# sailor-z/3DAHV

Measured on AMD Instinct MI355X. Metric: rotation hypotheses scored/sec (B=1), higher is better.
Workload: dtype f32; 1 GPU; CO3D pair (BASELINE.json configs[1]): B=1, ONE set of N_hyp=50000 Haar rotations split over the GPUs (contiguous shards, n_offset), source volume 16x8x8x8 (P=512 voxel sites x 16 ch), head 384->32->32, 64 positions; n_hyp_per_gpu=50000, n_hyp_total=50000, parallelism=hypothesis axis sharded x1, 8-byte key all-reduce(max), backend=single process, lanes=1

## Files before the change

### 3dahv_amd/_lib.py

```python
from __future__ import annotations

import ctypes
import os
import subprocess

_HERE = os.path.dirname(os.path.abspath(__file__))
CSRC = os.path.join(_HERE, "csrc")
LIB_PATH = os.path.join(CSRC, "libahv_hip.so")

AHV_SCORE_RESET_BEST = 1
AHV_SCORE_SPLIT_F16 = 2
AHV_SCORE_NO_TEAMS = 4
AHV_SCORE_SPARE_CUS_SHIFT = 8
AHV_SELECT_RESET_KEY = 1
AHV_KEY_EMPTY = -(1 << 63)
AHV_TOPK_MAX_K = 64
AHV_TOPK_RESET_LIST = 1
AHV_SO3_MAX_LADDER = 8
AHV_POSTERIOR_MAX_MODES = 16
AHV_POSTERIOR_RESET_STATE = 1
AHV_VIEWS_MAX = 16
AHV_VIEWS_RESET_BEST = 1
AHV_VIEWS_NO_ANGLE_LIMIT = 2
AHV_VIEW_SLOT_EXCLUDED = -1
AHV_VIEW_SLOT_OVERFLOW = -2

_vp = ctypes.c_void_p
_i64 = ctypes.c_int64
# ... 73 lines not shown
SIGNATURES["ahv_fuse_view_scores_compact_f32"] = (_int, [_vp, _vp, _vp, _int, _int, _i64, _i64, _i64, _vp, _vp, _u32, _vp])
SIGNATURES["ahv_resample_workspace_bytes"] = (ctypes.c_size_t, [_int, _i64])
SIGNATURES["ahv_resample_f32"] = (_int, [_vp, _int, _i64, ctypes.c_float, _i64, _vp, _vp, _vp, ctypes.c_size_t, _u32, _vp])
SIGNATURES["ahv_compose_rotations_indexed_f32"] = (_int, [_vp, _vp, _i64, _i64, _vp, _i64, _int, _vp, _vp])
SIGNATURES["ahv_diffuse_rotations_f32"] = (_int, [_vp, _vp, _i64, _i64, _vp, _i64, _i64, _int, ctypes.c_uint64, _vp, ctypes.c_float,
                                                  ctypes.c_float, _vp, _vp, _vp])
SIGNATURES["ahv_predict_rotations_f32"] = (_int, [_vp, _vp, _i64, _vp, _i64, _i64, _vp, _i64, _i64, _int, ctypes.c_uint64, _vp]
                                           + [ctypes.c_float] * 5 + [_int, _vp, _vp, _vp, _vp])
SIGNATURES["ahv_track_advance"] = (_int, [ctypes.c_uint64, _vp, _int, _vp, _vp])
SIGNATURES["ahv_smooth_step_f32"] = (_int, [_vp, _vp, _vp, _vp, _i64, _int, _i64, _i64] + [ctypes.c_float] * 4 + [_vp] * 5)
SIGNATURES["ahv_smooth_backtrace_f32"] = (_int, [_vp, _vp, _vp, _vp, _i64, _int, _i64, _i64, _i64, _vp, _vp, _vp])

DIAG_SIGNATURES = {
    "ahv_score_hypotheses_clocked_f32": SIGNATURES.pop("ahv_score_hypotheses_clocked_f32"),
    "ahv_diag_score_plan": (_int, [_int, _i64, _u32, ctypes.POINTER(_int), ctypes.POINTER(_int), ctypes.POINTER(_i64)]),
}

_lib = None


class AhvError(RuntimeError):
    """A libahv_hip call returned a negative status."""


def build(force: bool = False) -> str:
    args = ["make", "-C", CSRC, "-j4"] + (["-B"] if force else [])
    proc = subprocess.run(args, stdout=subprocess.PIPE, stderr=subprocess.STDOUT, text=True)
    if proc.returncode != 0:
        raise RuntimeError("building libahv_hip.so failed:\n" + proc.stdout)
    return LIB_PATH
# ... 26 lines not shown
```

### 3dahv_amd/csrc/ahv_abi.hip

```cpp
#include <hip/hip_runtime.h>

#include <cstdarg>
#include <cstdio>
#include <cstring>

#include "../../include/ahv.h"
#include "../../include/ahv_diag.h"
#include "ahv_launch.h"

namespace ahv {
hipError_t launch_unpack_best(const int64_t*, int, float*, int64_t*, hipStream_t);
hipError_t launch_rotate_volume(const float*, int64_t, const float*, int64_t, int, int, int, int, float*, int,
                                hipStream_t);
hipError_t launch_rotate_volume_backward(const float*, int64_t, const float*, int64_t, int, int, int, int, float*, int,
                                         hipStream_t);
hipError_t launch_forward_3d2d(const float*, const float*, const float*, const float*, int64_t, float*, int,
                               hipStream_t);
hipError_t launch_score_features(const float*, const float*, int, int64_t, float*, int, hipStream_t);
hipError_t launch_argmax(const float*, int, int64_t, int64_t, int64_t*, int, hipStream_t);
hipError_t launch_fill_keys(int64_t*, int, hipStream_t);
int topk_parts(int64_t N);
hipError_t launch_topk(const float*, int, int64_t, int64_t, int, int64_t*, int64_t*, bool, hipStream_t);
hipError_t launch_topk_merge(const int64_t*, int, int, int, int64_t*, bool, hipStream_t);
hipError_t launch_select_topk(int64_t*, int, const float*, int64_t, int64_t, int64_t, int, float*, float*, int64_t*, bool,
// ... 96 lines not shown

int ahv_device_cu_count(void)
{
    const int cu = cu_count();
    if (cu < 0) return fail(AHV_EDEVICE, "no usable HIP device");
    return cu;
}

static hipError_t zero_span(void* p, size_t bytes, hipStream_t s)
{
    void* const ptrs[1] = {p};
    const size_t n[1] = {bytes};
    return ahv::launch_zero_fill(ptrs, n, 1, s);
}

static int score_common(const char* who, const float* vol_src, const float* tgt, bool tgt_is_volume, const float* R,
                        int64_t r_batch_stride, int64_t n_offset, const float* W1, const float* W2, const float* b2, int B,
                        int64_t N, float* scores, int64_t* best_key, float* feat_tgt_out, unsigned flags,
                        uint64_t* clock_stamps, void* stream)
{
    if (B < 0 || N < 0) return fail(AHV_EINVAL, "%s: negative size (B=%d, N=%lld)", who, B, (long long)N);
    if (B > 0 && N > 0 && (!vol_src || !tgt || !R || !W1 || !W2 || !b2))
        return fail(AHV_EINVAL, "%s: null input pointer", who);
    if (r_batch_stride != 0 && r_batch_stride < N * 9)
        return fail(AHV_EINVAL, "%s: r_batch_stride %lld must be 0 or >= N*9", who, (long long)r_batch_stride);
    if (n_offset < 0 || n_offset + N > 4294967296ll)
        return fail(AHV_EINVAL, "%s: n_offset + N must fit in 32 bits", who);
    if (flags & ~(AHV_SCORE_RESET_BEST | AHV_SCORE_SPLIT_F16 | AHV_SCORE_NO_TEAMS | AHV_SCORE_SPARE_CUS_MASK))
        return fail(AHV_EINVAL, "%s: unknown flags 0x%x", who, flags);
    const bool split = (flags & AHV_SCORE_SPLIT_F16) != 0;
    hipStream_t s = static_cast<hipStream_t>(stream);
    if (best_key && (flags & AHV_SCORE_RESET_BEST) && B > 0) {
        hipError_t e = ahv::launch_fill_keys(best_key, B, s);
        if (e != hipSuccess) return hip_fail("score: key reset", e);
    }
    const int cu = cu_count();
    if (cu < 0) return fail(AHV_EDEVICE, "no usable HIP device");
    if (tgt_is_volume && split) {
        if (B > 0 && !feat_tgt_out)
            return fail(AHV_EINVAL, "%s: AHV_SCORE_SPLIT_F16 needs feat_tgt_out (the target features go through it)", who);
        if (B > 0) {
            hipError_t e = ahv::launch_forward_3d2d(tgt, W1, W2, b2, B, feat_tgt_out, cu, s);
            if (e != hipSuccess) return hip_fail("verify_pair: forward_3d2d launch", e);
        }
        tgt = feat_tgt_out;
        tgt_is_volume = false;
        feat_tgt_out = nullptr;
    }
    if (B == 0) return AHV_OK;
    if (N == 0 && !(tgt_is_volume && feat_tgt_out)) return AHV_OK;
    ahv::ScoreLaunch a;
    a.vol_src = vol_src; a.tgt = tgt; a.tgt_is_volume = tgt_is_volume; a.R = R;
    a.r_batch_stride = r_batch_stride; a.n_offset = n_offset; a.W1 = W1; a.W2 = W2; a.b2 = b2; a.B = B; a.N = N;
    a.scores = scores; a.best_key = best_key; a.feat_tgt_out = feat_tgt_out; a.num_cu = cu;
    a.spare_cu = (int)((flags & AHV_SCORE_SPARE_CUS_MASK) >> AHV_SCORE_SPARE_CUS_SHIFT);
    a.split_f16 = split; a.no_teams = (flags & AHV_SCORE_NO_TEAMS) != 0; a.clock_stamps = clock_stamps;
    hipError_t e = ahv::launch_score_hypotheses(a, s);
    if (e != hipSuccess) return hip_fail("score: launch", e);
    return AHV_OK;
}

int ahv_score_hypotheses_f32(const float* vol_src, const float* feat_tgt, const float* R,
                             int64_t r_batch_stride, int64_t n_offset, const float* W1, const float* W2,
                             const float* b2, int B, int64_t N, float* scores, int64_t* best_key,
                             unsigned flags, void* stream)
{
    return score_common("score", vol_src, feat_tgt, false, R, r_batch_stride, n_offset, W1, W2, b2, B, N, scores, best_key,
                        nullptr, flags, nullptr, stream);
}

int ahv_score_hypotheses_clocked_f32(const float* vol_src, const float* feat_tgt, const float* R,
// ... 5 lines not shown
    return score_common("score_clocked", vol_src, feat_tgt, false, R, r_batch_stride, n_offset, W1, W2, b2, B, N, scores,
                        best_key, nullptr, flags, clock_stamps, stream);
}

int ahv_diag_score_plan(int B, int64_t N, unsigned flags, int* gx, int* gy, int64_t* n_main)
{
    if (B < 1 || N < 0) return fail(AHV_EINVAL, "score_plan: bad shape (B=%d, N=%lld)", B, (long long)N);
    const int cu = cu_count();
    if (cu < 0) return fail(AHV_EDEVICE, "no usable HIP device");
    const bool teams = !(flags & AHV_SCORE_SPLIT_F16) && !(flags & AHV_SCORE_NO_TEAMS);
    const ahv::ScorePlan p = ahv::plan_score_launch(B, N, cu, (int)((flags & AHV_SCORE_SPARE_CUS_MASK) >> AHV_SCORE_SPARE_CUS_SHIFT), teams);
    if (gx) *gx = p.gx;
    if (gy) *gy = p.gy;
    if (n_main) *n_main = p.n_main;
    return AHV_OK;
}

int ahv_verify_pair_f32(const float* vol_src, const float* vol_tgt, const float* R, int64_t r_batch_stride,
                        int64_t n_offset, const float* W1, const float* W2, const float* b2, int B, int64_t N,
                        float* scores, int64_t* best_key, float* feat_tgt_out, unsigned flags, uint64_t* clock_stamps,
                        void* stream)
{
    return score_common("verify_pair", vol_src, vol_tgt, true, R, r_batch_stride, n_offset, W1, W2, b2, B, N, scores,
                        best_key, feat_tgt_out, flags, clock_stamps, stream);
}

int ahv_unpack_best(const int64_t* best_key, int B, float* best_score, int64_t* best_idx, void* stream)
{
    if (!best_key) return fail(AHV_EINVAL, "unpack: null best_key");
    if (B < 0) return fail(AHV_EINVAL, "unpack: negative B");
// ... 102 lines not shown

int ahv_coarse_to_fine_f32(const float* vol_src, const float* vol_tgt, const float* R, int64_t r_batch_stride, int64_t N,
                           const float* D, int64_t N2, const float* W1, const float* W2, const float* b2, int B,
                           float* scores_coarse, float* scores_fine, int64_t* keys, uint32_t* sync, float* feat_tgt_out,
                           float* R_pred, float* fine_score, int64_t* fine_idx, float* coarse_score, int64_t* coarse_idx,
                           unsigned flags, void* stream)
{
    if (B < 0 || N < 0 || N2 < 0) return fail(AHV_EINVAL, "coarse_to_fine: negative size (B=%d, N=%lld, N2=%lld)", B, (long long)N, (long long)N2);
    if (B == 0) return AHV_OK;
    if (N == 0 || N2 == 0) return fail(AHV_EINVAL, "coarse_to_fine: empty hypothesis set (N=%lld, N2=%lld)", (long long)N, (long long)N2);
    if (!vol_src || !vol_tgt || !R || !D || !W1 || !W2 || !b2) return fail(AHV_EINVAL, "coarse_to_fine: null input pointer");
    if (!keys || !sync) return fail(AHV_EINVAL, "coarse_to_fine: keys and sync are required (2 B keys, 2 B + 1 counters)");
    if (r_batch_stride != 0 && r_batch_stride < N * 9)
        return fail(AHV_EINVAL, "coarse_to_fine: r_batch_stride %lld must be 0 or >= N*9", (long long)r_batch_stride);
    if (N > 4294967296ll || N2 > 4294967296ll) return fail(AHV_EINVAL, "coarse_to_fine: indices must fit in 32 bits");
    if (flags & ~(AHV_SCORE_NO_TEAMS | AHV_SCORE_SPARE_CUS_MASK)) return fail(AHV_EINVAL, "coarse_to_fine: unknown flags 0x%x", flags);
    const int cu = cu_count();
    if (cu < 0) return fail(AHV_EDEVICE, "no usable HIP device");
    ahv::CoarseToFineLaunch a;
    ahv::ScoreLaunch& c = a.coarse;
    c.vol_src = vol_src; c.tgt = vol_tgt; c.tgt_is_volume = true; c.R = R; c.r_batch_stride = r_batch_stride; c.n_offset = 0;
    c.W1 = W1; c.W2 = W2; c.b2 = b2; c.B = B; c.N = N; c.scores = scores_coarse; c.best_key = keys;
    c.feat_tgt_out = feat_tgt_out; c.num_cu = cu;
    c.spare_cu = (int)((flags & AHV_SCORE_SPARE_CUS_MASK) >> AHV_SCORE_SPARE_CUS_SHIFT);
    c.split_f16 = false; c.no_teams = (flags & AHV_SCORE_NO_TEAMS) != 0; c.clock_stamps = nullptr;
    a.D = D; a.N2 = N2; a.scores2 = scores_fine; a.best_key2 = keys + B; a.sync = sync; a.R_pred = R_pred;
    a.fine_score = fine_score; a.coarse_score = coarse_score; a.fine_idx = fine_idx; a.coarse_idx = coarse_idx;
    hipError_t e = ahv::launch_coarse_to_fine(a, static_cast<hipStream_t>(stream));
    if (e != hipSuccess) return hip_fail("coarse_to_fine: launch", e);
    return AHV_OK;
}

int ahv_reset_best(int64_t* best_key, int B, void* stream)
{
    if (B < 0) return fail(AHV_EINVAL, "reset_best: negative B");
    if (B == 0) return AHV_OK;
    if (!best_key) return fail(AHV_EINVAL, "reset_best: null best_key");
    hipError_t e = ahv::launch_fill_keys(best_key, B, static_cast<hipStream_t>(stream));
    if (e != hipSuccess) return hip_fail("reset_best: launch", e);
    return AHV_OK;
// ... 746 lines not shown
```

### 3dahv_amd/csrc/ahv_launch.h

```cpp
#pragma once
#include <hip/hip_runtime.h>
#include <stdint.h>

namespace ahv {

struct ScoreLaunch {
    const float* vol_src;
    const float* tgt;
    bool tgt_is_volume;
    const float* R;
    int64_t r_batch_stride, n_offset;
    const float *W1, *W2, *b2;
    int B;
    int64_t N;
    float* scores;
    int64_t* best_key;
    float* feat_tgt_out;
    int num_cu, spare_cu;
    bool split_f16;
    bool no_teams;
    uint64_t* clock_stamps;
};

struct ScorePlan {
    int gx, gy;
    int64_t n_main;
};

ScorePlan plan_score_launch(int B, int64_t N, int num_cu, int spare_cu, bool teams);
hipError_t launch_score_hypotheses(const ScoreLaunch& a, hipStream_t stream);
hipError_t launch_score_hypotheses_train(const ScoreLaunch& a, float* u_out, hipStream_t stream);

struct CoarseToFineLaunch {
    ScoreLaunch coarse;
    const float* D;
    int64_t N2;
    float* scores2;
    int64_t* best_key2;
    uint32_t* sync;
    float* R_pred;
    float *fine_score, *coarse_score;
// ... 6 lines not shown
```

### 3dahv_amd/csrc/ahv_score.hip

```cpp
#define AHV_FP32_LOW_HALF
#include "ahv_dual.h"
#include "ahv_split.h"
#include "ahv_team.h"
#include "ahv_exact.h"
#include "ahv_launch.h"

namespace ahv {

__device__ __forceinline__ int opaque(int x)
{
    asm volatile("" : "+v"(x));
    return x;
}

__device__ __forceinline__ float swap_add32(float a, float b)
{
    const auto r = __builtin_amdgcn_permlane32_swap(__float_as_uint(a), __float_as_uint(b), false, false);
    return __uint_as_float(r[0]) + __uint_as_float(r[1]);
}

__device__ __forceinline__ float swap_add16(float a, float b)
{
    const auto r = __builtin_amdgcn_permlane16_swap(__float_as_uint(a), __float_as_uint(b), false, false);
    return __uint_as_float(r[0]) + __uint_as_float(r[1]);
// ... 147 lines not shown
            for (int m2 = 0; m2 < 2; ++m2)
                tg[t][m2] = *reinterpret_cast<const f32x4*>(lds_src + ((2 * t + m2) * 64 + lane) * kSrcStride + 16);
        const float s = hyp_score_rs<SPLIT || kFp32LowHalf>(v, tg, lane);
        if (scores_b != nullptr && lane == 0) scores_b[he] = s;
        const key_t key = pack_key(s, (unsigned)(n_offset + he));
        best = key > best ? key : best;
    }
    return best;
}

template <bool SPLIT, bool TGT, bool C2F, bool SAVE_U = false>
__device__ __forceinline__ void score_hypotheses_body(
    const float* __restrict__ vol_src, const float* __restrict__ tgt, const float* __restrict__ R,
    long r_batch_stride, long n_offset, const float* __restrict__ W1, const float* __restrict__ W2,
    const float* __restrict__ b2, int B, long N, long n_main, float* __restrict__ scores,
    key_t* __restrict__ best_key, float* __restrict__ feat_tgt_out, unsigned long long* __restrict__ clk, const C2fArgs& cf)
{
    static_assert(!(SPLIT && TGT), "the split-f16 kernel takes ready-made target features");
    static_assert(!C2F || (TGT && !SPLIT), "the two-stage launch is the fp32 verify kernel");
    static_assert(!SAVE_U || (!SPLIT && !TGT && !C2F), "u is saved by the fp32 scorer with ready-made target features");
    if constexpr (!SPLIT) asm volatile("" ::: "v255");
    __shared__ __attribute__((aligned(1024))) float lds_src[kSrcFloats];
    __shared__ __attribute__((aligned(16))) float lds_w1[kW1TableFloats];
    __shared__ __attribute__((aligned(16))) float lds_q[8 * kQuarterFloats];
    __shared__ TeamSync lds_team;
    __shared__ NonFinite lds_nf;
    __shared__ unsigned long long lds_t_entry[2];
    if (clk != nullptr && threadIdx.x == 0) {
        lds_t_entry[0] = __builtin_amdgcn_s_memrealtime();
        lds_t_entry[1] = __builtin_amdgcn_s_memtime();
    }
    const int tid = threadIdx.x;
// ... 248 lines not shown
                best = score_share_exact<SPLIT>(lds_src, lds_w1, buf, W1, W2, b2, Rb, ec, N_s, h0, hstep, sc_b, n_offset_s, best, lane);
            } else {
                best = score_share_exact<SPLIT>(lds_src, lds_w1, buf, W1, W2, b2, Rb, NoCompose{}, N_s, h0, hstep, sc_b, n_offset_s, best, lane);
            }
            if constexpr (SPLIT) split_load_resident(w1res, reinterpret_cast<const f16x8*>(lds_w1), lane);
            if constexpr (SAVE_U) {
                const f32x4 qn = f32x4{__builtin_nanf(""), __builtin_nanf(""), __builtin_nanf(""), __builtin_nanf("")};
                for (long he = h0; he < N_s; he += hstep) {
                    float* uo = feat_tgt_out + ((long)b * N_s + he) * 2048 + lane * 4;
#pragma unroll
                    for (int i = 0; i < 8; ++i) *reinterpret_cast<f32x4*>(uo + i * 256) = qn;
                }
            }
        } else {
        if constexpr (!SPLIT && !SAVE_U) score_remainder_by_teams();
        long h = (long)wave * gridDim.x + residue;
        float Rn = h < n_main_s ? Rb[h * 9 + rl] : 0.0f;
#ifdef AHV_STAMPS
        unsigned long long tsum[11] = {0, 0, 0, 0, 0, 0, 0, 0, 0, 0, 0};
#endif
        for (; h < n_main_s; h += hstep) {
            float Rm[9];
#pragma unroll
            for (int i = 0; i < 9; ++i) Rm[i] = __builtin_bit_cast(float, __builtin_amdgcn_readlane(__builtin_bit_cast(int, Rn), i));
            hyp_rotation(Rm, st1);
            {
                const long hn = (h + hstep < n_main_s) ? h + hstep : h;
                Rn = Rb[hn * 9 + rl];
            }
            f32x4 acc[2][4];
#pragma unroll
            for (int m = 0; m < 2; ++m)
#pragma unroll
                for (int t = 0; t < 4; ++t) acc[m][t] = f32x4{0.f, 0.f, 0.f, 0.f};

#ifdef AHV_STAMPS
            unsigned long long ts[11];
#define AHV_TS(i) AHV_STAMP(ts[i])
#else
#define AHV_TS(i)
#endif
            AHV_TS(0)
// ... 60 lines not shown
#pragma unroll
                for (int t = 0; t < 4; ++t)
#pragma unroll
                    for (int m2 = 0; m2 < 2; ++m2)
                        tg[t][m2] = *reinterpret_cast<const f32x4*>(lds_src + ((2 * t + m2) * 64 + lane) * kSrcStride + 16);
                s = hyp_score_rs<kFp32LowHalf>(v, tg, lane);
            }
            if (scores_s != nullptr && lane == 0) scores_s[(long)b * N_s + h] = s;
            const key_t key = pack_key(s, (unsigned)(n_offset_s + h));
            best = key > best ? key : best;
            AHV_TS(10)
#ifdef AHV_STAMPS
            for (int i = 0; i < 10; ++i) tsum[i] += ts[i + 1] - ts[i];
            tsum[10] += 1;
#endif
        }
#ifdef AHV_STAMPS
        if (lane == 0) {
            const int gw = (blockIdx.x * 8 + wave) & 2047;
            for (int i = 0; i < 11; ++i) g_stamps[gw * 16 + i] = tsum[i];
        }
#endif
        }
        if (key_s != nullptr && lane == 0 && best != kKeyEmpty) atomicMax(key_s + b, best);
      }
        ++samples_done;
        if (!SPLIT) {
            const int bn = b + (int)gridDim.y < B ? b + (int)gridDim.y : b;
            const int tid_e = wave * 64 + opaque(lane);
            src_regs_load(sv, vol_src + (long)bn * (16 * 512), tid_e);
            tgt_regs_load<TGT>(tv, tgt, bn, tid_e);
        }
        if constexpr (C2F) {
            __syncthreads();
            if (tid == 0) {
// ... 41 lines not shown
        if (wave == 0 && lane == 0) {
            unsigned long long* o = clk + 4 * (blockIdx.y * gridDim.x + blockIdx.x);
            o[0] = lds_t_entry[1];
            o[1] = lds_t_entry[0];
            o[2] = __builtin_amdgcn_s_memtime();
            o[3] = __builtin_amdgcn_s_memrealtime();
        }
    }
}

template <bool SPLIT, bool TGT>
__global__ __launch_bounds__(kDualThreads, 2) void score_hypotheses_dual_kernel(
    const float* __restrict__ vol_src, const float* __restrict__ tgt, const float* __restrict__ R,
    long r_batch_stride, long n_offset, const float* __restrict__ W1, const float* __restrict__ W2,
    const float* __restrict__ b2, int B, long N, long n_main, float* __restrict__ scores,
    key_t* __restrict__ best_key, float* __restrict__ feat_tgt_out, unsigned long long* __restrict__ clk)
{
    score_hypotheses_body<SPLIT, TGT, false>(vol_src, tgt, R, r_batch_stride, n_offset, W1, W2, b2, B, N, n_main, scores, best_key,
                                             feat_tgt_out, clk, C2fArgs{});
}

__global__ __launch_bounds__(kDualThreads, 2) void score_hypotheses_train_kernel(
    const float* __restrict__ vol_src, const float* __restrict__ tgt, const float* __restrict__ R,
    long r_batch_stride, const float* __restrict__ W1, const float* __restrict__ W2,
    const float* __restrict__ b2, int B, long N, float* __restrict__ scores, float* __restrict__ u_out)
{
    score_hypotheses_body<false, false, false, true>(vol_src, tgt, R, r_batch_stride, 0l, W1, W2, b2, B, N, N, scores, nullptr, u_out,
                                                     nullptr, C2fArgs{});
}

__global__ __launch_bounds__(kDualThreads, 2) void coarse_to_fine_kernel(
    const float* __restrict__ vol_src, const float* __restrict__ tgt, const float* __restrict__ R,
    long r_batch_stride, long n_offset, const float* __restrict__ W1, const float* __restrict__ W2,
    const float* __restrict__ b2, int B, long N, long n_main, float* __restrict__ scores,
    key_t* __restrict__ best_key, float* __restrict__ feat_tgt_out, C2fArgs cf)
{
    score_hypotheses_body<false, true, true>(vol_src, tgt, R, r_batch_stride, n_offset, W1, W2, b2, B, N, n_main, scores, best_key,
                                             feat_tgt_out, nullptr, cf);
}

__global__ void unpack_best_kernel(const key_t* __restrict__ best_key, int B, float* __restrict__ best_score,
                                   long* __restrict__ best_idx)
{
    const int b = blockIdx.x * blockDim.x + threadIdx.x;
    if (b >= B) return;
    const key_t k = best_key[b];
    if (best_score) best_score[b] = (k == kKeyEmpty) ? -INFINITY : key_score(k);
    if (best_idx) best_idx[b] = (k == kKeyEmpty) ? -1l : key_index(k);
}

}

namespace ahv {

ScorePlan plan_score_launch(int B, int64_t N, int num_cu, int spare_cu, bool teams)
{
    ScorePlan p;
    int avail = num_cu - spare_cu;
    if (avail < 1) avail = 1;
    p.gy = B < avail ? B : avail;
    if (p.gy < 1) p.gy = 1;
    int64_t gx = avail / p.gy;
    const int64_t want = teams ? (N + 1) / 2 : (N + 3) / 4;
    if (gx > want) gx = want;
    if (gx < 1) gx = 1;
    p.gx = (int)gx;
    const int64_t slots = 8 * gx, full = N / slots, rem = N - full * slots;
    p.n_main = (teams && rem > 0 && rem <= 2 * gx) ? full * slots : N;
    return p;
}

hipError_t launch_score_hypotheses(const ScoreLaunch& a, hipStream_t stream)
{
    static_assert(sizeof(key_t) == sizeof(int64_t), "key width");
    const bool teams = !a.split_f16 && !a.no_teams;
    const ScorePlan p = plan_score_launch(a.B, a.N, a.num_cu, a.spare_cu, teams);
    const dim3 grid(p.gx, p.gy), block(kDualThreads);
    auto* key = reinterpret_cast<key_t*>(a.best_key);
    auto* clk = reinterpret_cast<unsigned long long*>(a.clock_stamps);
    if (a.split_f16) {
        if (a.tgt_is_volume) return hipErrorInvalidValue;
        hipLaunchKernelGGL((score_hypotheses_dual_kernel<true, false>), grid, block, 0, stream, a.vol_src, a.tgt, a.R,
                           (long)a.r_batch_stride, (long)a.n_offset, a.W1, a.W2, a.b2, a.B, (long)a.N, (long)p.n_main, a.scores,
                           key, a.feat_tgt_out, clk);
    } else if (a.tgt_is_volume) {
        hipLaunchKernelGGL((score_hypotheses_dual_kernel<false, true>), grid, block, 0, stream, a.vol_src, a.tgt, a.R,
                           (long)a.r_batch_stride, (long)a.n_offset, a.W1, a.W2, a.b2, a.B, (long)a.N, (long)p.n_main, a.scores,
                           key, a.feat_tgt_out, clk);
    } else {
        hipLaunchKernelGGL((score_hypotheses_dual_kernel<false, false>), grid, block, 0, stream, a.vol_src, a.tgt, a.R,
                           (long)a.r_batch_stride, (long)a.n_offset, a.W1, a.W2, a.b2, a.B, (long)a.N, (long)p.n_main, a.scores,
                           key, a.feat_tgt_out, clk);
    }
    return hipGetLastError();
}

hipError_t launch_score_hypotheses_train(const ScoreLaunch& a, float* u_out, hipStream_t stream)
{
    if (a.split_f16 || a.tgt_is_volume || a.scores == nullptr || u_out == nullptr) return hipErrorInvalidValue;
    const ScorePlan p = plan_score_launch(a.B, a.N, a.num_cu, a.spare_cu, false);
    hipLaunchKernelGGL(score_hypotheses_train_kernel, dim3(p.gx, p.gy), dim3(kDualThreads), 0, stream, a.vol_src, a.tgt, a.R,
                       (long)a.r_batch_stride, a.W1, a.W2, a.b2, a.B, (long)a.N, a.scores, u_out);
    return hipGetLastError();
}

hipError_t launch_coarse_to_fine(const CoarseToFineLaunch& a, hipStream_t stream)
{
    const ScoreLaunch& c = a.coarse;
    const bool teams = !c.no_teams;
    const ScorePlan p = plan_score_launch(c.B, c.N, c.num_cu, c.spare_cu, teams);
    const int64_t slots = 8 * (int64_t)p.gx, full2 = a.N2 / slots, rem2 = a.N2 - full2 * slots;
    const int64_t n_main2 = (teams && rem2 > 0 && rem2 <= 2 * (int64_t)p.gx) ? full2 * slots : a.N2;
    if ((int64_t)p.gx * p.gy > c.num_cu) return hipErrorInvalidConfiguration;
    C2fArgs cf;
    cf.D = a.D;
    cf.N2 = (long)a.N2;
    cf.n_main2 = (long)n_main2;
    cf.best_key2 = reinterpret_cast<key_t*>(a.best_key2);
    cf.scores2 = a.scores2;
    cf.sync = a.sync;
    cf.R_pred = a.R_pred;
    cf.fine_score = a.fine_score;
    cf.coarse_score = a.coarse_score;
    cf.fine_idx = reinterpret_cast<long*>(a.fine_idx);
    cf.coarse_idx = reinterpret_cast<long*>(a.coarse_idx);
    hipLaunchKernelGGL(coarse_to_fine_kernel, dim3(p.gx, p.gy), dim3(kDualThreads), 0, stream, c.vol_src, c.tgt, c.R,
                       (long)c.r_batch_stride, (long)c.n_offset, c.W1, c.W2, c.b2, c.B, (long)c.N, (long)p.n_main, c.scores,
                       reinterpret_cast<key_t*>(c.best_key), c.feat_tgt_out, cf);
    return hipGetLastError();
}

hipError_t launch_unpack_best(const int64_t* best_key, int B, float* best_score, int64_t* best_idx,
                              hipStream_t stream)
{
    const int threads = 64;
    hipLaunchKernelGGL(unpack_best_kernel, dim3((B + threads - 1) / threads), dim3(threads), 0, stream,
                       reinterpret_cast<const key_t*>(best_key), B, best_score, reinterpret_cast<long*>(best_idx));
    return hipGetLastError();
}

}
```

### 3dahv_amd/ops.py

```python
from __future__ import annotations

import collections
import contextvars
import math
import struct

import torch

from . import _lib

_VOL = (16, 8, 8, 8)


_SPLIT_F16 = contextvars.ContextVar("ahv_split_f16", default=False)


class split_f16_scorer:

    def __init__(self, enabled: bool = True):
        self.enabled = bool(enabled)
        self._token = None

    def __enter__(self):
        self._token = _SPLIT_F16.set(self.enabled)
# ... 166 lines not shown
    B, N = scores.shape
    if N == 0:
        raise RuntimeError("max(): Expected reduction dim 1 to have non-zero size.")
    s = scores.detach().contiguous()
    key = torch.empty((B,), dtype=torch.int64, device=s.device)
    _call(key.device, "ahv_argmax_f32", s.data_ptr(), B, N, n_offset, key.data_ptr(), _lib.AHV_SCORE_RESET_BEST)
    if return_key:
        return key
    return unpack_best(key)


def score_hypotheses(vol_src: torch.Tensor, feat_tgt: torch.Tensor, R: torch.Tensor, W1: torch.Tensor,
                     W2: torch.Tensor, b2: torch.Tensor, n_offset: int = 0, want_scores: bool = True,
                     best_key: torch.Tensor | None = None, reset_best: bool | None = None,
                     split_f16: bool | None = None, clock_stamps: torch.Tensor | None = None,
                     no_teams: bool = False, spare_cus: int = 0):
    if (want_scores and clock_stamps is None and torch.is_grad_enabled()
            and any(t.requires_grad for t in (vol_src, feat_tgt, R, W1, W2, b2))):
        return _ScoreFn.apply(vol_src, feat_tgt, R, W1, W2, b2, n_offset, best_key, reset_best, split_f16)
    with torch.no_grad():
        return _score_hypotheses_nograd(vol_src, feat_tgt, R, W1, W2, b2, n_offset, want_scores, best_key, reset_best,
                                        split_f16, clock_stamps, no_teams=no_teams, spare_cus=spare_cus)


def score_plan(B: int, N: int, no_teams: bool = False, split_f16: bool = False, spare_cus: int = 0):
    import ctypes
    flags = ((_lib.AHV_SCORE_NO_TEAMS if no_teams else 0) | (_lib.AHV_SCORE_SPLIT_F16 if split_f16 else 0) |
             (int(spare_cus) << _lib.AHV_SCORE_SPARE_CUS_SHIFT))
    gx, gy, n_main = ctypes.c_int(), ctypes.c_int(), ctypes.c_int64()
    _lib.check(_lib.load().ahv_diag_score_plan(B, N, flags, ctypes.byref(gx), ctypes.byref(gy), ctypes.byref(n_main)),
               "ahv_diag_score_plan")
    return gx.value, gy.value, n_main.value


def verify_pair(vol_src: torch.Tensor, vol_tgt: torch.Tensor, R: torch.Tensor, W1: torch.Tensor, W2: torch.Tensor,
                b2: torch.Tensor, n_offset: int = 0, want_scores: bool = True, best_key: torch.Tensor | None = None,
                reset_best: bool | None = None, split_f16: bool | None = None, want_feat_tgt: bool = False,
                clock_stamps: torch.Tensor | None = None, no_teams: bool = False, spare_cus: int = 0,
                scores_out: torch.Tensor | None = None):
    _refuse_grad("verify_pair", vol_src, vol_tgt, R, W1, W2, b2)
    if vol_tgt.dim() != 5 or tuple(vol_tgt.shape) != tuple(vol_src.shape):
        raise RuntimeError("vol_tgt must have vol_src's shape (B,16,8,8,8), got %s" % (tuple(vol_tgt.shape),))
    split = bool(_SPLIT_F16.get() if split_f16 is None else split_f16)
    with torch.no_grad():
        feat = None
        if want_feat_tgt or split:
            feat = torch.empty((vol_src.shape[0], 32, 64), dtype=torch.float32, device=vol_src.device)
        scores, key = _score_hypotheses_nograd(vol_src, vol_tgt, R, W1, W2, b2, n_offset, want_scores, best_key, reset_best,
                                               split, clock_stamps, no_teams=no_teams, spare_cus=spare_cus,
                                               tgt_is_volume=True, feat_tgt_out=feat, scores_out=scores_out)
    return (scores, key, feat) if want_feat_tgt else (scores, key)


def _score_hypotheses_nograd(vol_src, feat_tgt, R, W1, W2, b2, n_offset, want_scores, best_key, reset_best, split_f16,
                             clock_stamps, no_teams=False, spare_cus=0, tgt_is_volume=False, feat_tgt_out=None, scores_out=None):
    if vol_src.dim() != 5 or tuple(vol_src.shape[1:]) != _VOL:
        raise RuntimeError("vol_src must be (B,16,8,8,8), got %s" % (tuple(vol_src.shape),))
    B = vol_src.shape[0]
    if not tgt_is_volume and tuple(feat_tgt.shape) != (B, 32, 64):
        raise RuntimeError("feat_tgt must be (B,32,64), got %s" % (tuple(feat_tgt.shape),))
    if R.dim() == 3 and tuple(R.shape[1:]) == (3, 3):
        N, rstride = R.shape[0], 0
    elif R.dim() == 4 and R.shape[0] == B and tuple(R.shape[2:]) == (3, 3):
        N, rstride = R.shape[1], R.shape[1] * 9
    else:
        raise RuntimeError("R must be (N,3,3) or (B,N,3,3), got %s" % (tuple(R.shape),))
    dev = _need_gpu(vol_src, feat_tgt, R, W1, W2, b2)
    W1, W2, b2 = _head(W1, W2, b2)
    vs, ft, Rc = vol_src.detach().contiguous(), feat_tgt.detach().contiguous(), R.detach().contiguous()
    scores = None
# ... 5 lines not shown
    elif want_scores:
        scores = torch.empty((B, N), dtype=torch.float32, device=dev)
    if best_key is None:
        best_key = torch.empty((B,), dtype=torch.int64, device=dev)
        reset_best = True
    elif best_key.dtype != torch.int64 or best_key.numel() != B or not best_key.is_cuda:
        raise RuntimeError("best_key must be a GPU int64 tensor of B elements")
    flags = _lib.AHV_SCORE_RESET_BEST if reset_best else 0
    if _SPLIT_F16.get() if split_f16 is None else split_f16:
        flags |= _lib.AHV_SCORE_SPLIT_F16
    if no_teams:
        flags |= _lib.AHV_SCORE_NO_TEAMS
    if not 0 <= int(spare_cus) <= 255:
        raise RuntimeError("spare_cus must be in 0..255")
    flags |= int(spare_cus) << _lib.AHV_SCORE_SPARE_CUS_SHIFT
    lib = _lib.load()
    head = (vs.data_ptr(), ft.data_ptr(), Rc.data_ptr(), rstride, n_offset, W1.data_ptr(), W2.data_ptr(), b2.data_ptr(),
            B, N, scores.data_ptr() if scores is not None else None, best_key.data_ptr())
    if clock_stamps is not None and (clock_stamps.dtype != torch.int64 or clock_stamps.device != dev or
                                     clock_stamps.numel() < 4 * lib.ahv_device_cu_count()):
        raise RuntimeError("clock_stamps must be an int64 tensor of 4 * CU-count elements on %s" % dev)
    with torch.cuda.device(dev):
        if tgt_is_volume:
            _lib.check(lib.ahv_verify_pair_f32(*head, feat_tgt_out.data_ptr() if feat_tgt_out is not None else None, flags,
                                               clock_stamps.data_ptr() if clock_stamps is not None else None,
                                               _stream(dev)), "ahv_verify_pair_f32")
        elif clock_stamps is None:
            _lib.check(lib.ahv_score_hypotheses_f32(*head, flags, _stream(dev)), "ahv_score_hypotheses_f32")
        else:
            _lib.check(lib.ahv_score_hypotheses_clocked_f32(*head, flags, clock_stamps.data_ptr(), _stream(dev)),
# ... 1270 lines not shown
            raise RuntimeError("3dahv_amd ops run on the GPU only (no CPU fallback); got device %s" % dev)
        self.B = B
        self.keys = torch.full((2, B), _lib.AHV_KEY_EMPTY, dtype=torch.int64, device=dev)
        self.sync = torch.zeros((2 * B + 1,), dtype=torch.int32, device=dev)

    def gave_up(self) -> bool:
        return bool(self.sync[-1].item() != 0)

    def clear_error(self) -> None:
        self.keys.fill_(_lib.AHV_KEY_EMPTY)
        self.sync.zero_()


def coarse_to_fine(vol_src: torch.Tensor, vol_tgt: torch.Tensor, R: torch.Tensor, D: torch.Tensor, W1: torch.Tensor,
                   W2: torch.Tensor, b2: torch.Tensor, state: CoarseToFineState | None = None, want_scores: bool = False,
                   want_feat_tgt: bool = False, no_teams: bool = False, spare_cus: int = 0, out: dict | None = None) -> dict:
    _refuse_grad("coarse_to_fine", vol_src, vol_tgt, W1, W2, b2)
    with torch.no_grad():
        return _coarse_to_fine_nograd(vol_src, vol_tgt, R, D, W1, W2, b2, state, want_scores, want_feat_tgt, no_teams,
                                      spare_cus, out)


def _coarse_to_fine_nograd(vol_src, vol_tgt, R, D, W1, W2, b2, state, want_scores, want_feat_tgt, no_teams, spare_cus, out):
    if vol_src.dim() != 5 or tuple(vol_src.shape[1:]) != _VOL or tuple(vol_tgt.shape) != tuple(vol_src.shape):
        raise RuntimeError("vol_src and vol_tgt must be (B,16,8,8,8), got %s and %s" % (tuple(vol_src.shape), tuple(vol_tgt.shape)))
    B = vol_src.shape[0]
    dev = _need_gpu(vol_src, vol_tgt, R, D, W1, W2, b2)
    N, rstride = _rot_layout(R, B)
    if D.dim() != 3 or tuple(D.shape[1:]) != (3, 3):
        raise RuntimeError("D must be (N2,3,3)")
    N2 = D.shape[0]
    W1, W2, b2 = _head(W1, W2, b2)
    if state is None:
        state = CoarseToFineState(B, dev)
    elif state.B != B or state.keys.device != dev:
        raise RuntimeError("the CoarseToFineState was made for B = %d on %s" % (state.B, state.keys.device))
    vs, vt, Rc, Dc = (t.detach().contiguous() for t in (vol_src, vol_tgt, R, D))
    o = out if out is not None else {}
    def buf(name, shape, dtype=torch.float32, wanted=True):
        if not wanted:
            return None
        if name not in o:
            o[name] = torch.empty(shape, dtype=dtype, device=dev)
        return o[name]
    sc = buf("coarse_scores", (B, N), wanted=want_scores)
    sf = buf("fine_scores", (B, N2), wanted=want_scores)
    ft = buf("feat_tgt", (B, 32, 64), wanted=want_feat_tgt)
    rp, fs, cs = buf("R_pred", (B, 3, 3)), buf("fine_score", (B,)), buf("coarse_score", (B,))
    fi, ci = buf("fine_idx", (B,), torch.int64), buf("coarse_idx", (B,), torch.int64)
    p = lambda t: 0 if t is None else t.data_ptr()
    if not 0 <= spare_cus <= 255:
        raise RuntimeError("spare_cus must be in [0, 255]")
    flags = (_lib.AHV_SCORE_NO_TEAMS if no_teams else 0) | (spare_cus << _lib.AHV_SCORE_SPARE_CUS_SHIFT)
    _call(dev, "ahv_coarse_to_fine_f32", vs.data_ptr(), vt.data_ptr(), Rc.data_ptr(), rstride, N, Dc.data_ptr(), N2,
          W1.data_ptr(), W2.data_ptr(), b2.data_ptr(), B, p(sc), p(sf), state.keys.data_ptr(), state.sync.data_ptr(), p(ft),
          rp.data_ptr(), fs.data_ptr(), fi.data_ptr(), cs.data_ptr(), ci.data_ptr(), flags)
    o["state"] = state
    return o


@torch.no_grad()
def so3_grid(n_total: int, device, offset: int = 0, n: int | None = None) -> torch.Tensor:
    n = n_total - offset if n is None else n
    out = torch.empty((n, 3, 3), dtype=torch.float32, device=device)
    if out.device.type != "cuda":
        raise RuntimeError("3dahv_amd ops run on the GPU only (no CPU fallback); got device %s" % out.device)
    _call(out.device, "ahv_so3_grid_f32", n_total, offset, n, out.data_ptr())
    return out
# ... 11 lines not shown
```

### include/ahv_diag.h

```cpp
#ifndef AHV_DIAG_H
#define AHV_DIAG_H

#include "ahv.h"

#ifdef __cplusplus
extern "C" {
#endif

#define AHV_SCORE_SPARE_CUS_SHIFT 8
#define AHV_SCORE_SPARE_CUS_MASK 0xFF00u
#define AHV_SCORE_SPARE_CUS(k) (((unsigned)(k) << AHV_SCORE_SPARE_CUS_SHIFT) & AHV_SCORE_SPARE_CUS_MASK)

int ahv_score_hypotheses_clocked_f32(const float* vol_src, const float* feat_tgt, const float* R,
                                     int64_t r_batch_stride, int64_t n_offset, const float* W1,
                                     const float* W2, const float* b2, int B, int64_t N, float* scores,
                                     int64_t* best_key, unsigned flags, uint64_t* clock_stamps, void* stream);

int ahv_diag_score_plan(int B, int64_t N, unsigned flags, int* gx, int* gy, int64_t* n_main);

#ifdef __cplusplus
}
#endif
#endif
```

Measured before the change: 73.01 million hypotheses/s.

## Deal hypotheses unevenly between wave halves with a 4:3 turn pattern

Replaces the fixed round-robin hypothesis stride in the fp32 scoring loop with a periodic 'deal' walk. Waves 0-3 and 4-7 of a workgroup take hypothesis slots in a 4:3 ratio, presumably because the two wave halves progress at different rates. The planner turns this on by default when each workgroup has enough hypotheses, and a flag lets callers force other ratios. The cost is extra per-iteration index arithmetic, plus a risk of tail imbalance if the assumed speed difference between the halves does not hold.

Measured after the change: 73.36 million hypotheses/s (median of 6 runs). Within noise of the previous version (+0.5%).

```diff
diff --git a/3dahv_amd/_lib.py b/3dahv_amd/_lib.py
--- a/3dahv_amd/_lib.py
+++ b/3dahv_amd/_lib.py
@@ -12,6 +12,7 @@
 AHV_SCORE_SPLIT_F16 = 2
 AHV_SCORE_NO_TEAMS = 4
 AHV_SCORE_SPARE_CUS_SHIFT = 8
+AHV_SCORE_DEAL_SHIFT = 16
 AHV_SELECT_RESET_KEY = 1
 AHV_KEY_EMPTY = -(1 << 63)
 AHV_TOPK_MAX_K = 64
@@ -115,6 +116,7 @@
 DIAG_SIGNATURES = {
     "ahv_score_hypotheses_clocked_f32": SIGNATURES.pop("ahv_score_hypotheses_clocked_f32"),
     "ahv_diag_score_plan": (_int, [_int, _i64, _u32, ctypes.POINTER(_int), ctypes.POINTER(_int), ctypes.POINTER(_i64)]),
+    "ahv_diag_score_deal": (_i64, [_i64, _int, _int, _int, _vp, _i64]),
 }
 
 _lib = None
diff --git a/3dahv_amd/csrc/ahv_abi.hip b/3dahv_amd/csrc/ahv_abi.hip
--- a/3dahv_amd/csrc/ahv_abi.hip
+++ b/3dahv_amd/csrc/ahv_abi.hip
@@ -134,6 +134,13 @@
     return ahv::launch_zero_fill(ptrs, n, 1, s);
 }
 
+static bool deal_from_flags(unsigned flags, int& a, int& b)
+{
+    a = (int)((flags >> AHV_SCORE_DEAL_SHIFT) & 15u);
+    b = (int)((flags >> (AHV_SCORE_DEAL_SHIFT + 4)) & 15u);
+    return (flags & AHV_SCORE_DEAL_MASK) == 0u || (a > 0 && b > 0);
+}
+
 static int score_common(const char* who, const float* vol_src, const float* tgt, bool tgt_is_volume, const float* R,
                         int64_t r_batch_stride, int64_t n_offset, const float* W1, const float* W2, const float* b2, int B,
                         int64_t N, float* scores, int64_t* best_key, float* feat_tgt_out, unsigned flags,
@@ -146,8 +153,11 @@
         return fail(AHV_EINVAL, "%s: r_batch_stride %lld must be 0 or >= N*9", who, (long long)r_batch_stride);
     if (n_offset < 0 || n_offset + N > 4294967296ll)
         return fail(AHV_EINVAL, "%s: n_offset + N must fit in 32 bits", who);
-    if (flags & ~(AHV_SCORE_RESET_BEST | AHV_SCORE_SPLIT_F16 | AHV_SCORE_NO_TEAMS | AHV_SCORE_SPARE_CUS_MASK))
+    if (flags & ~(AHV_SCORE_RESET_BEST | AHV_SCORE_SPLIT_F16 | AHV_SCORE_NO_TEAMS | AHV_SCORE_SPARE_CUS_MASK | AHV_SCORE_DEAL_MASK))
         return fail(AHV_EINVAL, "%s: unknown flags 0x%x", who, flags);
+    int deal_a, deal_b;
+    if (!deal_from_flags(flags, deal_a, deal_b))
+        return fail(AHV_EINVAL, "%s: AHV_SCORE_DEAL(%d, %d): both turn counts must be in 1..15", who, deal_a, deal_b);
     const bool split = (flags & AHV_SCORE_SPLIT_F16) != 0;
     hipStream_t s = static_cast<hipStream_t>(stream);
     if (best_key && (flags & AHV_SCORE_RESET_BEST) && B > 0) {
@@ -175,6 +185,7 @@
     a.scores = scores; a.best_key = best_key; a.feat_tgt_out = feat_tgt_out; a.num_cu = cu;
     a.spare_cu = (int)((flags & AHV_SCORE_SPARE_CUS_MASK) >> AHV_SCORE_SPARE_CUS_SHIFT);
     a.split_f16 = split; a.no_teams = (flags & AHV_SCORE_NO_TEAMS) != 0; a.clock_stamps = clock_stamps;
+    a.deal_a = deal_a; a.deal_b = deal_b;
     hipError_t e = ahv::launch_score_hypotheses(a, s);
     if (e != hipSuccess) return hip_fail("score: launch", e);
     return AHV_OK;
@@ -210,6 +221,20 @@
     if (gy) *gy = p.gy;
     if (n_main) *n_main = p.n_main;
     return AHV_OK;
+}
+
+int64_t ahv_diag_score_deal(int64_t K, int a, int b, int wave, int64_t* idx, int64_t capacity)
+{
+    if (K < 0 || a < 1 || b < 1 || a > ahv::kDealMaxTurns || b > ahv::kDealMaxTurns || wave < 0 || wave > 7 || capacity < 0 ||
+        (capacity > 0 && !idx))
+        return fail(AHV_EINVAL, "score_deal: bad argument (K=%lld, a=%d, b=%d, wave=%d)", (long long)K, a, b, wave);
+    ahv::DealWalk walk;
+    int64_t n = 0;
+    for (int64_t k = ahv::deal_first(walk, ahv::deal_upper_mask(a, b), a + b, wave); k < K; k += ahv::deal_step(walk)) {
+        if (n < capacity) idx[n] = k;
+        ++n;
+    }
+    return n;
 }
 
 int ahv_verify_pair_f32(const float* vol_src, const float* vol_tgt, const float* R, int64_t r_batch_stride,
@@ -342,7 +367,11 @@
     if (r_batch_stride != 0 && r_batch_stride < N * 9)
         return fail(AHV_EINVAL, "coarse_to_fine: r_batch_stride %lld must be 0 or >= N*9", (long long)r_batch_stride);
     if (N > 4294967296ll || N2 > 4294967296ll) return fail(AHV_EINVAL, "coarse_to_fine: indices must fit in 32 bits");
-    if (flags & ~(AHV_SCORE_NO_TEAMS | AHV_SCORE_SPARE_CUS_MASK)) return fail(AHV_EINVAL, "coarse_to_fine: unknown flags 0x%x", flags);
+    if (flags & ~(AHV_SCORE_NO_TEAMS | AHV_SCORE_SPARE_CUS_MASK | AHV_SCORE_DEAL_MASK))
+        return fail(AHV_EINVAL, "coarse_to_fine: unknown flags 0x%x", flags);
+    int deal_a, deal_b;
+    if (!deal_from_flags(flags, deal_a, deal_b))
+        return fail(AHV_EINVAL, "coarse_to_fine: AHV_SCORE_DEAL(%d, %d): both turn counts must be in 1..15", deal_a, deal_b);
     const int cu = cu_count();
     if (cu < 0) return fail(AHV_EDEVICE, "no usable HIP device");
     ahv::CoarseToFineLaunch a;
@@ -352,6 +381,7 @@
     c.feat_tgt_out = feat_tgt_out; c.num_cu = cu;
     c.spare_cu = (int)((flags & AHV_SCORE_SPARE_CUS_MASK) >> AHV_SCORE_SPARE_CUS_SHIFT);
     c.split_f16 = false; c.no_teams = (flags & AHV_SCORE_NO_TEAMS) != 0; c.clock_stamps = nullptr;
+    c.deal_a = deal_a; c.deal_b = deal_b;
     a.D = D; a.N2 = N2; a.scores2 = scores_fine; a.best_key2 = keys + B; a.sync = sync; a.R_pred = R_pred;
     a.fine_score = fine_score; a.coarse_score = coarse_score; a.fine_idx = fine_idx; a.coarse_idx = coarse_idx;
     hipError_t e = ahv::launch_coarse_to_fine(a, static_cast<hipStream_t>(stream));
diff --git a/3dahv_amd/csrc/ahv_launch.h b/3dahv_amd/csrc/ahv_launch.h
--- a/3dahv_amd/csrc/ahv_launch.h
+++ b/3dahv_amd/csrc/ahv_launch.h
@@ -20,11 +20,54 @@
     bool split_f16;
     bool no_teams;
     uint64_t* clock_stamps;
+    int deal_a, deal_b;
 };
+
+constexpr int kDealMaxTurns = 15;
+
+__host__ __device__ inline unsigned deal_upper_mask(int a, int b)
+{
+    unsigned m = 0;
+    for (int t = 0, e = 0; t < a + b; ++t) {
+        e += b;
+        if (e >= a + b) {
+            e -= a + b;
+            m |= 1u << t;
+        }
+    }
+    return m;
+}
+
+struct DealWalk {
+    unsigned mask;
+    int period;
+    int t;
+};
+
+__host__ __device__ inline int deal_first(DealWalk& w, unsigned upper_mask, int period, int wave)
+{
+    w.mask = wave >= 4 ? upper_mask : ~upper_mask & ((1u << period) - 1u);
+    w.period = period;
+    w.t = __builtin_ctz(w.mask);
+    return 4 * w.t + (wave & 3);
+}
+
+__host__ __device__ inline int deal_step(DealWalk& w)
+{
+    const unsigned rest = w.mask >> (w.t + 1);
+    const int t0 = w.t;
+    w.t = rest != 0u ? t0 + 1 + __builtin_ctz(rest) : __builtin_ctz(w.mask);
+    return 4 * (rest != 0u ? w.t - t0 : w.t - t0 + w.period);
+}
+
+constexpr int kDealA = 4, kDealB = 3;
+constexpr int kDealMinPeriods = 5;
+inline bool deal_pays(int64_t per_workgroup) { return per_workgroup >= (int64_t)kDealMinPeriods * 4 * (kDealA + kDealB); }
 
 struct ScorePlan {
     int gx, gy;
     int64_t n_main;
+    int deal_a, deal_b;
 };
 
 ScorePlan plan_score_launch(int B, int64_t N, int num_cu, int spare_cu, bool teams);
diff --git a/3dahv_amd/csrc/ahv_score.hip b/3dahv_amd/csrc/ahv_score.hip
--- a/3dahv_amd/csrc/ahv_score.hip
+++ b/3dahv_amd/csrc/ahv_score.hip
@@ -185,8 +185,10 @@
     const float* __restrict__ vol_src, const float* __restrict__ tgt, const float* __restrict__ R,
     long r_batch_stride, long n_offset, const float* __restrict__ W1, const float* __restrict__ W2,
     const float* __restrict__ b2, int B, long N, long n_main, float* __restrict__ scores,
-    key_t* __restrict__ best_key, float* __restrict__ feat_tgt_out, unsigned long long* __restrict__ clk, const C2fArgs& cf)
-{
+    key_t* __restrict__ best_key, float* __restrict__ feat_tgt_out, unsigned long long* __restrict__ clk, const C2fArgs& cf,
+    unsigned deal_upper = 2u, int deal_period = 2)
+{
+    constexpr bool DEAL = !SPLIT && !SAVE_U;
     static_assert(!(SPLIT && TGT), "the split-f16 kernel takes ready-made target features");
     static_assert(!C2F || (TGT && !SPLIT), "the two-stage launch is the fp32 verify kernel");
     static_assert(!SAVE_U || (!SPLIT && !TGT && !C2F), "u is saved by the fp32 scorer with ready-made target features");
@@ -465,18 +467,26 @@
             }
         } else {
         if constexpr (!SPLIT && !SAVE_U) score_remainder_by_teams();
-        long h = (long)wave * gridDim.x + residue;
+        DealWalk walk = {0u, 0, 0};
+        long h;
+        if constexpr (DEAL) h = (long)deal_first(walk, deal_upper, deal_period, wave) * gridDim.x + residue;
+        else h = (long)wave * gridDim.x + residue;
         float Rn = h < n_main_s ? Rb[h * 9 + rl] : 0.0f;
 #ifdef AHV_STAMPS
         unsigned long long tsum[11] = {0, 0, 0, 0, 0, 0, 0, 0, 0, 0, 0};
 #endif
-        for (; h < n_main_s; h += hstep) {
+        for (bool more = h < n_main_s; more;) {
             float Rm[9];
 #pragma unroll
             for (int i = 0; i < 9; ++i) Rm[i] = __builtin_bit_cast(float, __builtin_amdgcn_readlane(__builtin_bit_cast(int, Rn), i));
             hyp_rotation(Rm, st1);
+            long h_next;
+            if constexpr (DEAL) h_next = h + (long)deal_step(walk) * gridDim.x;
+            else h_next = h + hstep;
+            if constexpr (DEAL) more = (long)((unsigned long)n_main_s - 1ul - (unsigned long)h_next) >= 0;
+            else more = h_next < n_main_s;
             {
-                const long hn = (h + hstep < n_main_s) ? h + hstep : h;
+                const long hn = more ? h_next : h;
                 Rn = Rb[hn * 9 + rl];
             }
             f32x4 acc[2][4];
@@ -567,11 +577,14 @@
             for (int i = 0; i < 10; ++i) tsum[i] += ts[i + 1] - ts[i];
             tsum[10] += 1;
 #endif
+            h = h_next;
         }
 #ifdef AHV_STAMPS
         if (lane == 0) {
             const int gw = (blockIdx.x * 8 + wave) & 2047;
             for (int i = 0; i < 11; ++i) g_stamps[gw * 16 + i] = tsum[i];
+            g_stamps[gw * 16 + 11] = __builtin_amdgcn_s_memrealtime();
+            g_stamps[gw * 16 + 12] = wg_t_loop;
         }
 #endif
         }
@@ -643,10 +656,11 @@
     const float* __restrict__ vol_src, const float* __restrict__ tgt, const float* __restrict__ R,
     long r_batch_stride, long n_offset, const float* __restrict__ W1, const float* __restrict__ W2,
     const float* __restrict__ b2, int B, long N, long n_main, float* __restrict__ scores,
-    key_t* __restrict__ best_key, float* __restrict__ feat_tgt_out, unsigned long long* __restrict__ clk)
+    key_t* __restrict__ best_key, float* __restrict__ feat_tgt_out, unsigned long long* __restrict__ clk,
+    unsigned deal_upper, int deal_period)
 {
     score_hypotheses_body<SPLIT, TGT, false>(vol_src, tgt, R, r_batch_stride, n_offset, W1, W2, b2, B, N, n_main, scores, best_key,
-                                             feat_tgt_out, clk, C2fArgs{});
+                                             feat_tgt_out, clk, C2fArgs{}, deal_upper, deal_period);
 }
 
 __global__ __launch_bounds__(kDualThreads, 2) void score_hypotheses_train_kernel(
@@ -662,10 +676,10 @@
     const float* __restrict__ vol_src, const float* __restrict__ tgt, const float* __restrict__ R,
     long r_batch_stride, long n_offset, const float* __restrict__ W1, const float* __restrict__ W2,
     const float* __restrict__ b2, int B, long N, long n_main, float* __restrict__ scores,
-    key_t* __restrict__ best_key, float* __restrict__ feat_tgt_out, C2fArgs cf)
+    key_t* __restrict__ best_key, float* __restrict__ feat_tgt_out, C2fArgs cf, unsigned deal_upper, int deal_period)
 {
     score_hypotheses_body<false, true, true>(vol_src, tgt, R, r_batch_stride, n_offset, W1, W2, b2, B, N, n_main, scores, best_key,
-                                             feat_tgt_out, nullptr, cf);
+                                             feat_tgt_out, nullptr, cf, deal_upper, deal_period);
 }
 
 __global__ void unpack_best_kernel(const key_t* __restrict__ best_key, int B, float* __restrict__ best_score,
@@ -696,7 +710,18 @@
     p.gx = (int)gx;
     const int64_t slots = 8 * gx, full = N / slots, rem = N - full * slots;
     p.n_main = (teams && rem > 0 && rem <= 2 * gx) ? full * slots : N;
+    const bool uneven = deal_pays(p.n_main / gx);
+    p.deal_a = uneven ? kDealA : 1;
+    p.deal_b = uneven ? kDealB : 1;
     return p;
+}
+
+static void launch_deal(const ScoreLaunch& a, const ScorePlan& p, unsigned& upper, int& period)
+{
+    const bool forced = a.deal_a > 0 && a.deal_b > 0;
+    const int da = forced ? a.deal_a : p.deal_a, db = forced ? a.deal_b : p.deal_b;
+    upper = deal_upper_mask(da, db);
+    period = da + db;
 }
 
 hipError_t launch_score_hypotheses(const ScoreLaunch& a, hipStream_t stream)
@@ -707,19 +732,24 @@
     const dim3 grid(p.gx, p.gy), block(kDualThreads);
     auto* key = reinterpret_cast<key_t*>(a.best_key);
     auto* clk = reinterpret_cast<unsigned long long*>(a.clock_stamps);
+    if (a.deal_a < 0 || a.deal_b < 0 || a.deal_a > kDealMaxTurns || a.deal_b > kDealMaxTurns || (a.deal_a == 0) != (a.deal_b == 0))
+        return hipErrorInvalidValue;
+    unsigned upper;
+    int period;
+    launch_deal(a, p, upper, period);
     if (a.split_f16) {
         if (a.tgt_is_volume) return hipErrorInvalidValue;
         hipLaunchKernelGGL((score_hypotheses_dual_kernel<true, false>), grid, block, 0, stream, a.vol_src, a.tgt, a.R,
                            (long)a.r_batch_stride, (long)a.n_offset, a.W1, a.W2, a.b2, a.B, (long)a.N, (long)p.n_main, a.scores,
-                           key, a.feat_tgt_out, clk);
+                           key, a.feat_tgt_out, clk, 2u, 2);
     } else if (a.tgt_is_volume) {
         hipLaunchKernelGGL((score_hypotheses_dual_kernel<false, true>), grid, block, 0, stream, a.vol_src, a.tgt, a.R,
                            (long)a.r_batch_stride, (long)a.n_offset, a.W1, a.W2, a.b2, a.B, (long)a.N, (long)p.n_main, a.scores,
-                           key, a.feat_tgt_out, clk);
+                           key, a.feat_tgt_out, clk, upper, period);
     } else {
         hipLaunchKernelGGL((score_hypotheses_dual_kernel<false, false>), grid, block, 0, stream, a.vol_src, a.tgt, a.R,
                            (long)a.r_batch_stride, (long)a.n_offset, a.W1, a.W2, a.b2, a.B, (long)a.N, (long)p.n_main, a.scores,
-                           key, a.feat_tgt_out, clk);
+                           key, a.feat_tgt_out, clk, upper, period);
     }
     return hipGetLastError();
 }
@@ -741,6 +771,13 @@
     const int64_t slots = 8 * (int64_t)p.gx, full2 = a.N2 / slots, rem2 = a.N2 - full2 * slots;
     const int64_t n_main2 = (teams && rem2 > 0 && rem2 <= 2 * (int64_t)p.gx) ? full2 * slots : a.N2;
     if ((int64_t)p.gx * p.gy > c.num_cu) return hipErrorInvalidConfiguration;
+    if (c.deal_a < 0 || c.deal_b < 0 || c.deal_a > kDealMaxTurns || c.deal_b > kDealMaxTurns || (c.deal_a == 0) != (c.deal_b == 0))
+        return hipErrorInvalidValue;
+    unsigned upper;
+    int period;
+    ScorePlan pd = p;
+    if (!deal_pays(n_main2 / p.gx)) pd.deal_a = pd.deal_b = 1;
+    launch_deal(c, pd, upper, period);
     C2fArgs cf;
     cf.D = a.D;
     cf.N2 = (long)a.N2;
@@ -755,7 +792,7 @@
     cf.coarse_idx = reinterpret_cast<long*>(a.coarse_idx);
     hipLaunchKernelGGL(coarse_to_fine_kernel, dim3(p.gx, p.gy), dim3(kDualThreads), 0, stream, c.vol_src, c.tgt, c.R,
                        (long)c.r_batch_stride, (long)c.n_offset, c.W1, c.W2, c.b2, c.B, (long)c.N, (long)p.n_main, c.scores,
-                       reinterpret_cast<key_t*>(c.best_key), c.feat_tgt_out, cf);
+                       reinterpret_cast<key_t*>(c.best_key), c.feat_tgt_out, cf, upper, period);
     return hipGetLastError();
 }
 
diff --git a/3dahv_amd/ops.py b/3dahv_amd/ops.py
--- a/3dahv_amd/ops.py
+++ b/3dahv_amd/ops.py
@@ -204,13 +204,13 @@
                      W2: torch.Tensor, b2: torch.Tensor, n_offset: int = 0, want_scores: bool = True,
                      best_key: torch.Tensor | None = None, reset_best: bool | None = None,
                      split_f16: bool | None = None, clock_stamps: torch.Tensor | None = None,
-                     no_teams: bool = False, spare_cus: int = 0):
+                     no_teams: bool = False, spare_cus: int = 0, deal: tuple[int, int] | None = None):
     if (want_scores and clock_stamps is None and torch.is_grad_enabled()
             and any(t.requires_grad for t in (vol_src, feat_tgt, R, W1, W2, b2))):
         return _ScoreFn.apply(vol_src, feat_tgt, R, W1, W2, b2, n_offset, best_key, reset_best, split_f16)
     with torch.no_grad():
         return _score_hypotheses_nograd(vol_src, feat_tgt, R, W1, W2, b2, n_offset, want_scores, best_key, reset_best,
-                                        split_f16, clock_stamps, no_teams=no_teams, spare_cus=spare_cus)
+                                        split_f16, clock_stamps, no_teams=no_teams, spare_cus=spare_cus, deal=deal)
 
 
 def score_plan(B: int, N: int, no_teams: bool = False, split_f16: bool = False, spare_cus: int = 0):
@@ -223,11 +223,20 @@
     return gx.value, gy.value, n_main.value
 
 
+def _deal_flags(deal) -> int:
+    if deal is None:
+        return 0
+    a, b = (int(x) for x in deal)
+    if not (1 <= a <= 15 and 1 <= b <= 15):
+        raise RuntimeError("deal must be (a, b) with both in 1..15")
+    return (a | (b << 4)) << _lib.AHV_SCORE_DEAL_SHIFT
+
+
 def verify_pair(vol_src: torch.Tensor, vol_tgt: torch.Tensor, R: torch.Tensor, W1: torch.Tensor, W2: torch.Tensor,
                 b2: torch.Tensor, n_offset: int = 0, want_scores: bool = True, best_key: torch.Tensor | None = None,
                 reset_best: bool | None = None, split_f16: bool | None = None, want_feat_tgt: bool = False,
                 clock_stamps: torch.Tensor | None = None, no_teams: bool = False, spare_cus: int = 0,
-                scores_out: torch.Tensor | None = None):
+                scores_out: torch.Tensor | None = None, deal: tuple[int, int] | None = None):
     _refuse_grad("verify_pair", vol_src, vol_tgt, R, W1, W2, b2)
     if vol_tgt.dim() != 5 or tuple(vol_tgt.shape) != tuple(vol_src.shape):
         raise RuntimeError("vol_tgt must have vol_src's shape (B,16,8,8,8), got %s" % (tuple(vol_tgt.shape),))
@@ -238,12 +247,13 @@
             feat = torch.empty((vol_src.shape[0], 32, 64), dtype=torch.float32, device=vol_src.device)
         scores, key = _score_hypotheses_nograd(vol_src, vol_tgt, R, W1, W2, b2, n_offset, want_scores, best_key, reset_best,
                                                split, clock_stamps, no_teams=no_teams, spare_cus=spare_cus,
-                                               tgt_is_volume=True, feat_tgt_out=feat, scores_out=scores_out)
+                                               tgt_is_volume=True, feat_tgt_out=feat, scores_out=scores_out, deal=deal)
     return (scores, key, feat) if want_feat_tgt else (scores, key)
 
 
 def _score_hypotheses_nograd(vol_src, feat_tgt, R, W1, W2, b2, n_offset, want_scores, best_key, reset_best, split_f16,
-                             clock_stamps, no_teams=False, spare_cus=0, tgt_is_volume=False, feat_tgt_out=None, scores_out=None):
+                             clock_stamps, no_teams=False, spare_cus=0, tgt_is_volume=False, feat_tgt_out=None, scores_out=None,
+                             deal=None):
     if vol_src.dim() != 5 or tuple(vol_src.shape[1:]) != _VOL:
         raise RuntimeError("vol_src must be (B,16,8,8,8), got %s" % (tuple(vol_src.shape),))
     B = vol_src.shape[0]
@@ -279,6 +289,7 @@
     if not 0 <= int(spare_cus) <= 255:
         raise RuntimeError("spare_cus must be in 0..255")
     flags |= int(spare_cus) << _lib.AHV_SCORE_SPARE_CUS_SHIFT
+    flags |= _deal_flags(deal)
     lib = _lib.load()
     head = (vs.data_ptr(), ft.data_ptr(), Rc.data_ptr(), rstride, n_offset, W1.data_ptr(), W2.data_ptr(), b2.data_ptr(),
             B, N, scores.data_ptr() if scores is not None else None, best_key.data_ptr())
@@ -1579,14 +1590,15 @@
 
 def coarse_to_fine(vol_src: torch.Tensor, vol_tgt: torch.Tensor, R: torch.Tensor, D: torch.Tensor, W1: torch.Tensor,
                    W2: torch.Tensor, b2: torch.Tensor, state: CoarseToFineState | None = None, want_scores: bool = False,
-                   want_feat_tgt: bool = False, no_teams: bool = False, spare_cus: int = 0, out: dict | None = None) -> dict:
+                   want_feat_tgt: bool = False, no_teams: bool = False, spare_cus: int = 0, out: dict | None = None,
+                   deal: tuple[int, int] | None = None) -> dict:
     _refuse_grad("coarse_to_fine", vol_src, vol_tgt, W1, W2, b2)
     with torch.no_grad():
         return _coarse_to_fine_nograd(vol_src, vol_tgt, R, D, W1, W2, b2, state, want_scores, want_feat_tgt, no_teams,
-                                      spare_cus, out)
-
-
-def _coarse_to_fine_nograd(vol_src, vol_tgt, R, D, W1, W2, b2, state, want_scores, want_feat_tgt, no_teams, spare_cus, out):
+                                      spare_cus, out, deal)
+
+
+def _coarse_to_fine_nograd(vol_src, vol_tgt, R, D, W1, W2, b2, state, want_scores, want_feat_tgt, no_teams, spare_cus, out, deal=None):
     if vol_src.dim() != 5 or tuple(vol_src.shape[1:]) != _VOL or tuple(vol_tgt.shape) != tuple(vol_src.shape):
         raise RuntimeError("vol_src and vol_tgt must be (B,16,8,8,8), got %s and %s" % (tuple(vol_src.shape), tuple(vol_tgt.shape)))
     B = vol_src.shape[0]
@@ -1616,7 +1628,7 @@
     p = lambda t: 0 if t is None else t.data_ptr()
     if not 0 <= spare_cus <= 255:
         raise RuntimeError("spare_cus must be in [0, 255]")
-    flags = (_lib.AHV_SCORE_NO_TEAMS if no_teams else 0) | (spare_cus << _lib.AHV_SCORE_SPARE_CUS_SHIFT)
+    flags = (_lib.AHV_SCORE_NO_TEAMS if no_teams else 0) | (spare_cus << _lib.AHV_SCORE_SPARE_CUS_SHIFT) | _deal_flags(deal)
     _call(dev, "ahv_coarse_to_fine_f32", vs.data_ptr(), vt.data_ptr(), Rc.data_ptr(), rstride, N, Dc.data_ptr(), N2,
           W1.data_ptr(), W2.data_ptr(), b2.data_ptr(), B, p(sc), p(sf), state.keys.data_ptr(), state.sync.data_ptr(), p(ft),
           rp.data_ptr(), fs.data_ptr(), fi.data_ptr(), cs.data_ptr(), ci.data_ptr(), flags)
diff --git a/include/ahv_diag.h b/include/ahv_diag.h
--- a/include/ahv_diag.h
+++ b/include/ahv_diag.h
@@ -11,6 +11,10 @@
 #define AHV_SCORE_SPARE_CUS_MASK 0xFF00u
 #define AHV_SCORE_SPARE_CUS(k) (((unsigned)(k) << AHV_SCORE_SPARE_CUS_SHIFT) & AHV_SCORE_SPARE_CUS_MASK)
 
+#define AHV_SCORE_DEAL_SHIFT 16
+#define AHV_SCORE_DEAL_MASK 0xFF0000u
+#define AHV_SCORE_DEAL(a, b) (((((unsigned)(a) & 15u) | (((unsigned)(b) & 15u) << 4)) << AHV_SCORE_DEAL_SHIFT) & AHV_SCORE_DEAL_MASK)
+
 int ahv_score_hypotheses_clocked_f32(const float* vol_src, const float* feat_tgt, const float* R,
                                      int64_t r_batch_stride, int64_t n_offset, const float* W1,
                                      const float* W2, const float* b2, int B, int64_t N, float* scores,
@@ -18,6 +22,8 @@
 
 int ahv_diag_score_plan(int B, int64_t N, unsigned flags, int* gx, int* gy, int64_t* n_main);
 
+int64_t ahv_diag_score_deal(int64_t K, int a, int b, int wave, int64_t* idx, int64_t capacity);
+
 #ifdef __cplusplus
 }
 #endif
```
